# dalab/matrix-manifolds

Hardware: AMD Instinct MI355X
Metric: pairwise manifold-dist/sec (fwd+bwd), SPD(3) 5k-node (higher is better)
Workload: dtype f32; 1 GPU; grqc-class graph, n=5000 nodes -> SPD(3) affine-invariant, all 12497500 pairs, squared distance + backward, reference init (||log X||=0.1); parallelism=pair-rows sharded x1, 1 all-reduce, launch=hipGraph replay (kernels)

## Files before the change

matrix-manifolds_amd/csrc/smallmat.hpp:

```cpp
#pragma once
#include <hip/hip_runtime.h>

#include <cstdint>
#include <type_traits>
#include <utility>

namespace mm {

template <int D> struct Packed { static constexpr int NP = D * (D + 1) / 2; };

__host__ __device__ constexpr int pidx(int r, int c) {
  return r >= c ? r * (r + 1) / 2 + c : c * (c + 1) / 2 + r;
}

template <typename T> struct Num;
template <> struct Num<float> {
  static __device__ __forceinline__ float eps() { return 5.9604645e-8f; }
  static __device__ __forceinline__ float tiny() { return 1e-37f; }
  static __device__ __forceinline__ float sqrt(float x) { return __builtin_amdgcn_sqrtf(x); }
  static __device__ __forceinline__ float rsqrt(float x) { return __builtin_amdgcn_rsqf(x); }
  static __device__ __forceinline__ float rcp(float x) { return __builtin_amdgcn_rcpf(x); }
  static __device__ __forceinline__ float rcp_fast(float x) { return __builtin_amdgcn_rcpf(x); }
  static __device__ __forceinline__ float log(float x) { return __builtin_amdgcn_logf(x) * 0.6931471805599453f; }
  static __device__ __forceinline__ float exp(float x) { return ::expf(x); }
// ... 318 lines not shown
        const T apq = a[pidx(q, p)];
        const T h = a[pidx(q, q)] - a[pidx(p, p)];
        const T ah = N::abs(h) + T(1e-15);
        const T sa_ = (h < T(0)) ? -apq : apq;
        const T sa2 = sa_ + sa_;
        const T r = N::rsqrt(N::fma(ah, ah, sa2 * sa2));
        const T x = N::fma(ah * r, T(0.5), T(0.5));
        const T ci = N::rsqrt(x);
        const T c = x * ci;
        const T s = (sa_ * r) * ci;
        const T t = s * ci;
        a[pidx(p, p)] = N::fma(-t, apq, a[pidx(p, p)]);
        a[pidx(q, q)] = N::fma(t, apq, a[pidx(q, q)]);
        a[pidx(q, p)] = T(0);
#pragma unroll
        for (int r2 = 0; r2 < D; ++r2) {
          if (r2 == p || r2 == q) continue;
          const T arp = a[pidx(r2, p)], arq = a[pidx(r2, q)];
          a[pidx(r2, p)] = N::fma(c, arp, -s * arq);
          a[pidx(r2, q)] = N::fma(s, arp, c * arq);
        }
        if (WITH_V) {
#pragma unroll
          for (int r2 = 0; r2 < D; ++r2) {
            const T vrp = v[r2][p], vrq = v[r2][q];
            v[r2][p] = N::fma(c, vrp, -s * vrq);
            v[r2][q] = N::fma(s, vrp, c * vrq);
          }
        }
      }
    }
  }
}
template <typename T, int D, bool WITH_V>
__device__ __forceinline__ void jacobi_eig(T (&a)[Packed<D>::NP], T (&v)[D][D]) {
  jacobi_eig<T, D, WITH_V>(a, v, Num<T>::eps() * Num<T>::eps());
}

template <typename T, int D, bool WITH_V>
__device__ __forceinline__ void svd_onesided(const T (&g)[D][D], T (&b)[D][D], T (&v)[D][D], T tol2) {
  using N = Num<T>;
#pragma unroll
  for (int r = 0; r < D; ++r)
#pragma unroll
    for (int c = 0; c < D; ++c) {
      b[r][c] = g[r][c];
      if (WITH_V) v[r][c] = (r == c) ? T(1) : T(0);
    }
  if constexpr (D == 1) return;
  for (int sweep = 0; sweep < N::kMaxSweeps + 4; ++sweep) {
    bool active = false;
#pragma unroll
    for (int p = 0; p < D - 1; ++p) {
#pragma unroll
      for (int q = p + 1; q < D; ++q) {
        T app = T(0), aqq = T(0), apq = T(0);
#pragma unroll
        for (int r = 0; r < D; ++r) {
          app = N::fma(b[r][p], b[r][p], app);
          aqq = N::fma(b[r][q], b[r][q], aqq);
          apq = N::fma(b[r][p], b[r][q], apq);
        }
        active = active || (apq * apq > tol2 * (app * aqq));
        const T h = aqq - app;
        const T ah = N::abs(h) + T(1e-15);
        const T sa_ = (h < T(0)) ? -apq : apq;
        const T sa2 = sa_ + sa_;
        const T rr = N::rsqrt(N::fma(ah, ah, sa2 * sa2));
        const T x = N::fma(ah * rr, T(0.5), T(0.5));
        const T ci = N::rsqrt(x);
        const T c = x * ci;
        const T sn = (sa_ * rr) * ci;
#pragma unroll
        for (int r = 0; r < D; ++r) {
          const T bp = b[r][p], bq = b[r][q];
          b[r][p] = N::fma(c, bp, -sn * bq);
          b[r][q] = N::fma(sn, bp, c * bq);
          if (WITH_V) {
            const T vp = v[r][p], vq = v[r][q];
            v[r][p] = N::fma(c, vp, -sn * vq);
            v[r][q] = N::fma(sn, vp, c * vq);
          }
        }
      }
    }
    if (!__any(active)) break;
  }
}

__device__ __forceinline__ void eig3_trig(const float (&a)[6], float (&w)[3]) {
  const float q = (a[pidx(0, 0)] + a[pidx(1, 1)] + a[pidx(2, 2)]) * (1.f / 3.f);
  const float b00 = a[pidx(0, 0)] - q, b11 = a[pidx(1, 1)] - q, b22 = a[pidx(2, 2)] - q;
  const float o10 = a[pidx(1, 0)], o20 = a[pidx(2, 0)], o21 = a[pidx(2, 1)];
  float p2 = fmaf(b00, b00, fmaf(b11, b11, b22 * b22));
  p2 = fmaf(2.f, fmaf(o10, o10, fmaf(o20, o20, o21 * o21)), p2) * (1.f / 6.f);
  const float ip = __builtin_amdgcn_rsqf(fmaxf(p2, 1e-30f));
  const float p = p2 * ip;
  const float c00 = b00 * ip, c11 = b11 * ip, c22 = b22 * ip, c10 = o10 * ip, c20 = o20 * ip, c21 = o21 * ip;
  float hd = c00 * fmaf(c11, c22, -c21 * c21) - c10 * fmaf(c10, c22, -c21 * c20) + c20 * fmaf(c10, c21, -c11 * c20);
  hd = fminf(fmaxf(0.5f * hd, -1.f), 1.f);
  const float ax = fabsf(hd);
  float pa = fmaf(-0.0012624911f, ax, 0.0066700901f);
  pa = fmaf(pa, ax, -0.0170881256f);
  pa = fmaf(pa, ax, 0.0308918810f);
  pa = fmaf(pa, ax, -0.0501743046f);
  pa = fmaf(pa, ax, 0.0889789874f);
  pa = fmaf(pa, ax, -0.2145988016f);
  pa = fmaf(pa, ax, 1.5707963050f);
  const float ac = __builtin_amdgcn_sqrtf(1.f - ax) * pa;
  const float phi = ((hd < 0.f) ? 3.14159265358979f - ac : ac) * (1.f / 3.f);
  const float z = phi * phi;
  float cs = fmaf(z, -2.7557319e-7f, 2.4801587e-5f);
  cs = fmaf(cs, z, -1.3888889e-3f);
  cs = fmaf(cs, z, 4.1666667e-2f);
  cs = fmaf(cs, z, -0.5f);
  cs = fmaf(cs, z, 1.f);
  float sn = fmaf(z, -2.5052108e-8f, 2.7557319e-6f);
  sn = fmaf(sn, z, -1.9841270e-4f);
  sn = fmaf(sn, z, 8.3333333e-3f);
  sn = fmaf(sn, z, -1.6666667e-1f);
  sn = fmaf(sn * z, phi, phi);
  const float r3s = 1.7320508f * sn;
  w[2] = fmaf(p, cs + cs, q);
  w[1] = fmaf(p, r3s - cs, q);
  w[0] = fmaf(p, -r3s - cs, q);
}

template <typename T> struct LogSeries;
template <> struct LogSeries<float> {
  static constexpr int kTerms = 8;
  static constexpr float kA[kTerms] = {9.999999337e-01f, -4.999999402e-01f, 3.333568549e-01f, -2.500212282e-01f,
                                       1.987095623e-01f, -1.655023071e-01f, 1.650813480e-01f, -1.450413880e-01f};
  static constexpr float at(int i) { return kA[i]; }
};
template <> struct LogSeries<double> {
  static constexpr int kTerms = 20;
  static constexpr double kA[kTerms] = {
    1.00000000000000000e+00, -4.99999999999999944e-01, 3.33333333333343085e-01, -2.50000000000014155e-01,
    1.99999999996232608e-01, -1.66666666663750795e-01, 1.42857143404437337e-01, -1.25000000386766896e-01,
    1.11111071374215928e-01, -9.99999703591583217e-02, 9.09107326619259803e-02, -8.33346464041358065e-02,
    7.68821017515587124e-02, -7.13938378893102243e-02, 6.72936081364212679e-02, -6.30553787420979894e-02,
    5.31216751520414421e-02, -5.03380364382464973e-02, 8.02156472153527783e-02, -7.58480457039158590e-02};
  static constexpr double at(int i) { return kA[i]; }
};

template <typename T> __device__ __forceinline__ T log_series3(const T (&a)[6], T (&m0)[6], T pre = T(1)) {
  using N = Num<T>;
  using S = LogSeries<T>;
  const T e00 = a[pidx(0, 0)] - T(1), e11 = a[pidx(1, 1)] - T(1), e22 = a[pidx(2, 2)] - T(1);
  const T e10 = a[pidx(1, 0)], e20 = a[pidx(2, 0)], e21 = a[pidx(2, 1)];
  const T f00 = N::fma(e00, e00, N::fma(e10, e10, e20 * e20));
  const T f11 = N::fma(e10, e10, N::fma(e11, e11, e21 * e21));
  const T f22 = N::fma(e20, e20, N::fma(e21, e21, e22 * e22));
  const T f10 = N::fma(e10, e00, N::fma(e11, e10, e21 * e20));
  const T f20 = N::fma(e20, e00, N::fma(e21, e10, e22 * e20));
  const T f21 = N::fma(e20, e10, N::fma(e21, e11, e22 * e21));
  const T tr2 = f00 + f11 + f22;
  const T s1 = e00 + e11 + e22;
  const T s2 = T(0.5) * N::fma(s1, s1, -tr2);
  const T s3 = e00 * N::fma(e11, e22, -e21 * e21) - e10 * N::fma(e10, e22, -e21 * e20) +
               e20 * N::fma(e10, e21, -e11 * e20);
  T a0, a1, a2;
  ring_horner3<T, S>(s1, s2, s3, a0, a1, a2);
  const T b0 = (a2 * s3) * pre, b1 = N::fma(-a2, s2, a0) * pre, b2 = N::fma(a2, s1, a1) * pre;
  m0[pidx(0, 0)] = N::fma(b2, f00, N::fma(b1, e00, b0));
  m0[pidx(1, 1)] = N::fma(b2, f11, N::fma(b1, e11, b0));
  m0[pidx(2, 2)] = N::fma(b2, f22, N::fma(b1, e22, b0));
  m0[pidx(1, 0)] = N::fma(b2, f10, b1 * e10);
  m0[pidx(2, 0)] = N::fma(b2, f20, b1 * e20);
  m0[pidx(2, 1)] = N::fma(b2, f21, b1 * e21);
  return tr2;
}

constexpr double kCentredGate3 = 0.6534;
template <typename T> struct LogSeriesWide;
template <> struct LogSeriesWide<float> {
  static constexpr int kTerms = 16;
  static constexpr float kA[kTerms] = {9.999999847e-01f, -4.999999854e-01f, 3.333378158e-01f, -2.500042795e-01f,
                                       1.997873233e-01f, -1.664636323e-01f, 1.466440033e-01f, -1.286147090e-01f,
                                       7.866430935e-02f, -6.903477397e-02f, 2.371349367e-01f, -2.228347962e-01f,
                                       -2.667691364e-01f, 2.562672116e-01f, 4.274908187e-01f, -4.061057313e-01f};
  static constexpr float at(int i) { return kA[i]; }
};
template <> struct LogSeriesWide<double> {
  static constexpr int kTerms = 36;
  static constexpr double kA[kTerms] = {
    0.999999999999999977, -0.499999999999999978, 0.333333333333367457, -0.250000000000033421,
    0.199999999991592943, -0.166666666658432825, 0.142857143675747047, -0.125000000801733994,
    0.111111069196670012, -0.0999999589496586145, 0.0909103925504135392, -0.0833346081274524372,
    0.0768964148318060428, -0.071402459598029521, 0.0670466571631664423, -0.0628721421125401977,
    0.054920735255657598, -0.0517334464941176604, 0.0821825618685663011, -0.0789393499687729317,
    -0.119544506131984601, 0.11824425305853179, 0.753586818196905653, -0.737031529750978713,
    -2.21838624927452971, 2.17293423563498954, 5.34587266623974133, -5.23378983222008806,
    -8.94716963622682544, 8.7602754349000368, 10.4325804141314891, -10.2127945466777319,
    -7.42237802920880408, 7.26540890455107326, 2.58226980159039129, -2.52672226697783483};
  static constexpr double at(int i) { return kA[i]; }
};
template <typename T> __device__ __forceinline__ bool centred_far3(const T (&a)[6]) {
  using N = Num<T>;
  const T mu = (a[pidx(0, 0)] + a[pidx(1, 1)] + a[pidx(2, 2)]) * T(1.0 / 3.0);
  const T d0 = a[pidx(0, 0)] - mu, d1 = a[pidx(1, 1)] - mu, d2 = a[pidx(2, 2)] - mu;
  const T off = N::fma(a[pidx(1, 0)], a[pidx(1, 0)], N::fma(a[pidx(2, 0)], a[pidx(2, 0)], a[pidx(2, 1)] * a[pidx(2, 1)]));
  const T dev = N::fma(d0, d0, N::fma(d1, d1, N::fma(d2, d2, off + off)));
  return !(dev <= T(kCentredGate3) * (mu * mu)) || !(mu > T(0));
}
template <typename T> __device__ __forceinline__ void log_series3_centred(const T (&a)[6], T (&m0)[6], T pre = T(1)) {
  using N = Num<T>;
  using S = LogSeriesWide<T>;
  const T mu = (a[pidx(0, 0)] + a[pidx(1, 1)] + a[pidx(2, 2)]) * T(1.0 / 3.0);
  const T rmu = N::rcp(mu);
  const T e00 = N::fma(a[pidx(0, 0)], rmu, T(-1)), e11 = N::fma(a[pidx(1, 1)], rmu, T(-1)), e22 = N::fma(a[pidx(2, 2)], rmu, T(-1));
  const T e10 = a[pidx(1, 0)] * rmu, e20 = a[pidx(2, 0)] * rmu, e21 = a[pidx(2, 1)] * rmu;
  const T f00 = N::fma(e00, e00, N::fma(e10, e10, e20 * e20));
  const T f11 = N::fma(e10, e10, N::fma(e11, e11, e21 * e21));
  const T f22 = N::fma(e20, e20, N::fma(e21, e21, e22 * e22));
  const T f10 = N::fma(e10, e00, N::fma(e11, e10, e21 * e20));
  const T f20 = N::fma(e20, e00, N::fma(e21, e10, e22 * e20));
  const T f21 = N::fma(e20, e10, N::fma(e21, e11, e22 * e21));
  const T s2 = T(-0.5) * (f00 + f11 + f22);
  const T s3 = e00 * N::fma(e11, e22, -e21 * e21) - e10 * N::fma(e10, e22, -e21 * e20) +
               e20 * N::fma(e10, e21, -e11 * e20);
  T a0, a1, a2;
  ring_horner3<T, S, true>(T(0), s2, s3, a0, a1, a2);
  const T logmu = N::log(mu);
  const T b0 = N::fma(a2, s3, logmu) * pre, b1 = N::fma(-a2, s2, a0) * pre, b2 = a1 * pre;
  m0[pidx(0, 0)] = N::fma(b2, f00, N::fma(b1, e00, b0));
  m0[pidx(1, 1)] = N::fma(b2, f11, N::fma(b1, e11, b0));
  m0[pidx(2, 2)] = N::fma(b2, f22, N::fma(b1, e22, b0));
  m0[pidx(1, 0)] = N::fma(b2, f10, b1 * e10);
  m0[pidx(2, 0)] = N::fma(b2, f20, b1 * e20);
  m0[pidx(2, 1)] = N::fma(b2, f21, b1 * e21);
}

template <typename T> struct LogSqSeriesWide;
template <> struct LogSqSeriesWide<float> {
  static constexpr int kTerms = 16;
  static constexpr float kQ[kTerms] = {9.999998930e-01f, -9.999998963e-01f, 9.166980138e-01f, -8.333637039e-01f,
                                       7.596244972e-01f, -6.985597554e-01f, 6.746606801e-01f, -6.295878238e-01f,
                                       3.395295792e-01f, -3.133767555e-01f, 1.520582314e+00f, -1.462563750e+00f,
                                       -1.927056128e+00f, 1.871837175e+00f, 2.893810986e+00f, -2.795949233e+00f};
  static constexpr float at(int i) { return kQ[i]; }
};
template <typename T> __device__ __forceinline__ T logsq_series3_centred(const T (&a)[6]) {
  using N = Num<T>;
  using S = LogSqSeriesWide<T>;
  const T mu = (a[pidx(0, 0)] + a[pidx(1, 1)] + a[pidx(2, 2)]) * T(1.0 / 3.0);
  const T rmu = N::rcp(mu);
  const T e00 = N::fma(a[pidx(0, 0)], rmu, T(-1)), e11 = N::fma(a[pidx(1, 1)], rmu, T(-1)), e22 = N::fma(a[pidx(2, 2)], rmu, T(-1));
  const T e10 = a[pidx(1, 0)] * rmu, e20 = a[pidx(2, 0)] * rmu, e21 = a[pidx(2, 1)] * rmu;
  T t2 = N::fma(e00, e00, N::fma(e11, e11, e22 * e22));
  t2 = N::fma(T(2), N::fma(e10, e10, N::fma(e20, e20, e21 * e21)), t2);
  const T s1 = e00 + e11 + e22;
  const T s2 = T(-0.5) * t2;
  const T s3 = e00 * N::fma(e11, e22, -e21 * e21) - e10 * N::fma(e10, e22, -e21 * e20) +
               e20 * N::fma(e10, e21, -e11 * e20);
  T h0, h1, h2;
  ring_horner3<T, S, true>(T(0), s2, s3, h0, h1, h2);
  const T core = N::fma(h2, T(0.5) * t2 * t2, N::fma(h1, T(3) * s3, h0 * t2));
  const T lmu = N::log(mu), ldet = N::log((T(1) + s1) + (s2 + s3));
  return N::fma(lmu, N::fma(T(3), lmu, ldet + ldet), core);
}

constexpr double kCayleyGate = 0.36;
template <typename T> __device__ __forceinline__ T frexp_t(T x, int* k);
template <> __device__ __forceinline__ float frexp_t<float>(float x, int* k) { return ::frexpf(x, k); }
template <> __device__ __forceinline__ double frexp_t<double>(double x, int* k) { return ::frexp(x, k); }
template <typename T> __device__ __forceinline__ T ldexp_t(T x, int k);
template <> __device__ __forceinline__ float ldexp_t<float>(float x, int k) { return ::ldexpf(x, k); }
template <> __device__ __forceinline__ double ldexp_t<double>(double x, int k) { return ::ldexp(x, k); }

template <typename T> struct CayleyP;
template <> struct CayleyP<float> {
  static constexpr int K = 6;
  static constexpr float c[K + 1] = {1.00000002318570891e+00f, 3.33327042495924375e-01f, 2.00274867564608688e-01f,
                                     1.38428695737667723e-01f, 1.44240977093542333e-01f, -3.05379184438951401e-02f,
                                     2.73482843603638170e-01f};
  static constexpr int kTerms = K + 1;
  static constexpr float at(int i) { return c[i]; }
};
template <> struct CayleyP<double> {
  static constexpr int K = 13;
  static constexpr double c[K + 1] = {9.99999999999997002e-01, 3.33333333336093829e-01, 1.99999999512113669e-01,
                                      1.42857176992888746e-01, 1.11109865194520263e-01, 9.09362522505209464e-02,
                                      7.65413194323763535e-02, 7.02835946952955759e-02, 3.51739351378960174e-02,
                                      1.60038305495638411e-01, -2.87332526616183470e-01, 7.35063731671786291e-01,
                                      -8.29196169410508666e-01, 5.70221868872885063e-01};
  static constexpr int kTerms = K + 1;
  static constexpr double at(int i) { return c[i]; }
};
constexpr double kCayleyNarrow = 0.16;
struct CayleyPn64 {
  static constexpr double c[10] = {0.999999999999997828, 0.333333333336045998, 0.199999999442592788, 0.142857187137109386,
                                   0.111109332105236778, 0.0909499162581166662, 0.0763574513803657068, 0.0714494792571264998,
                                   0.0350458696353453726, 0.113663386241058913};
  static constexpr int kTerms = 10;
  static constexpr double at(int i) { return c[i]; }
};
struct CayleyQn64 {
  static constexpr double c[11] = {1.00000000000000037, 0.666666666666100058, 0.511111111252317187, 0.419047605361109196,
                                   0.357460995535957299, 0.313015598858362064, 0.279652848994267891, 0.248774877825649445,
                                   0.25954346018603201, 0.0906375847139156082, 0.475855998018695552};
  static constexpr int kTerms = 11;
  static constexpr double at(int i) { return c[i]; }
};
template <typename T> __device__ __forceinline__ T cayley_scale(T mean, T* logmu) {
  int k;
  const T mant = frexp_t<T>(mean, &k);
  if (mant < T(0.70710678118654752)) k -= 1;
  *logmu = T(k) * T(0.69314718055994531);
  return ldexp_t<T>(T(1), -k);
}
template <typename T>
__device__ __forceinline__ void cayley3_spectrum(T s1, T s2, T s3, T& rD, T& z1, T& z2, T& z3, T& t1, T& t2, T& t3) {
  using N = Num<T>;
  const T s33 = T(3) * s3;
  rD = N::rcp_fast(N::fma(T(4), s1, T(8)) + N::fma(T(2), s2, s3));
  z1 = N::fma(T(4), s1 + s2, s33) * rD;
  z2 = N::fma(T(2), s2, s33) * rD;
  z3 = s3 * rD;
  t1 = N::fma(z1, z1, T(-2) * z2);
  t2 = N::fma(z2, z2, T(-2) * (z1 * z3));
  t3 = z3 * z3;
}
template <typename T> __device__ __forceinline__ T log_cayley3(const T (&a)[6], T (&m0)[6], T pre = T(1)) {
  using N = Num<T>;
  using P = CayleyP<T>;
  T logmu;
  const T r = cayley_scale<T>((a[0] + a[2] + a[5]) * T(1.0 / 3.0), &logmu);
  const T e00 = N::fma(a[0], r, T(-1)), e11 = N::fma(a[2], r, T(-1)), e22 = N::fma(a[5], r, T(-1));
  const T e10 = a[1] * r, e20 = a[3] * r, e21 = a[4] * r;
  const T f00 = N::fma(e00, e00, N::fma(e10, e10, e20 * e20));
  const T f11 = N::fma(e10, e10, N::fma(e11, e11, e21 * e21));
  const T f22 = N::fma(e20, e20, N::fma(e21, e21, e22 * e22));
  const T f10 = N::fma(e10, e00, N::fma(e11, e10, e21 * e20));
  const T f20 = N::fma(e20, e00, N::fma(e21, e10, e22 * e20));
  const T f21 = N::fma(e20, e10, N::fma(e21, e11, e22 * e21));
  const T s1 = e00 + e11 + e22;
  const T s2 = T(0.5) * N::fma(s1, s1, -(f00 + f11 + f22));
  const T s3 = e00 * N::fma(e11, e22, -e21 * e21) - e10 * N::fma(e10, e22, -e21 * e20) +
               e20 * N::fma(e10, e21, -e11 * e20);
  T rD, z1, z2, z3, t1, t2, t3;
  cayley3_spectrum<T>(s1, s2, s3, rD, z1, z2, z3, t1, t2, t3);
  T c0, c1, c2;
  if constexpr (std::is_same<T, double>::value) {
    if (!__any(!(t1 <= T(kCayleyNarrow)))) ring_horner3<T, CayleyPn64>(t1, t2, t3, c0, c1, c2);
    else ring_horner3<T, P>(t1, t2, t3, c0, c1, c2);
  } else {
    ring_horner3<T, P>(t1, t2, t3, c0, c1, c2);
  }
  T b0 = c2 * z3, b1 = N::fma(-c2, z2, c1), b2 = c2 * z1;
  {
    const T n0 = N::fma(b2, z3, c0), n1 = N::fma(-b2, z2, b0), n2 = N::fma(b2, z1, b1);
    b0 = n0; b1 = n1; b2 = n2;
  }
  {
    const T n0 = b2 * z3, n1 = N::fma(-b2, z2, b0), n2 = N::fma(b2, z1, b1);
    b0 = n0; b1 = n1; b2 = n2;
  }
  const T y0 = z3, y2 = T(-2) * rD, y1 = -(s1 + T(2)) * y2;
  const T q0 = y0 * y0, q1 = T(2) * (y0 * y1), q2 = N::fma(T(2) * y0, y2, y1 * y1), q3 = T(2) * (y1 * y2), q4 = y2 * y2;
  const T h2 = N::fma(s1, s1, -s2), h1 = N::fma(-s1, s2, s3), h0 = s1 * s3;
  const T w0 = N::fma(q4, h0, N::fma(q3, s3, q0));
  const T w1 = N::fma(q4, h1, N::fma(-q3, s2, q1));
  const T w2 = N::fma(q4, h2, N::fma(q3, s1, q2));
  const T p2 = pre + pre;
  const T g0 = N::fma(N::fma(b2, w0, N::fma(b1, y0, b0)), p2, logmu * pre);
  const T g1 = N::fma(b2, w1, b1 * y1) * p2;
  const T g2 = N::fma(b2, w2, b1 * y2) * p2;
  m0[0] = N::fma(g2, f00, N::fma(g1, e00, g0));
  m0[2] = N::fma(g2, f11, N::fma(g1, e11, g0));
  m0[5] = N::fma(g2, f22, N::fma(g1, e22, g0));
  m0[1] = N::fma(g2, f10, g1 * e10);
  m0[3] = N::fma(g2, f20, g1 * e20);
  m0[4] = N::fma(g2, f21, g1 * e21);
  return t1;
}

template <typename T> struct CayleyQ;
template <> struct CayleyQ<float> {
  static constexpr int K = 7;
  static constexpr float c[K + 1] = {0.999999990659938783f, 0.666669978862739941f, 0.510920481665167664f, 0.423174655546735851f,
                                     0.314332175292986808f, 0.551201736862719326f, -0.412567514510121138f, 1.17039095371423926f};
  static constexpr int kTerms = K + 1;
  static constexpr float at(int i) { return c[i]; }
};
template <> struct CayleyQ<double> {
  static constexpr int K = 15;
  static constexpr double c[K + 1] = {0.99999999999999987, 0.666666666666851142, 0.511111111067702619, 0.419047623073864087,
                                      0.35746012197040091, 0.313040831979712641, 0.279195466546191997, 0.254162482860379539,
                                      0.217779908930427374, 0.303497422045376885, -0.242356046115491071, 1.74002823450430709,
                                      -3.70667784316895825, 6.72451540777742607, -6.69607770346690423, 3.64458881905822882};
  static constexpr int kTerms = K + 1;
  static constexpr double at(int i) { return c[i]; }
};
template <typename T> __device__ __forceinline__ T logsq_cayley3(const T (&a)[6], T logdet_a, T* gate) {
  using N = Num<T>;
  using Q = CayleyQ<T>;
  T logmu;
  const T r = cayley_scale<T>((a[0] + a[2] + a[5]) * T(1.0 / 3.0), &logmu);
  const T e00 = N::fma(a[0], r, T(-1)), e11 = N::fma(a[2], r, T(-1)), e22 = N::fma(a[5], r, T(-1));
  const T e10 = a[1] * r, e20 = a[3] * r, e21 = a[4] * r;
  const T s1 = e00 + e11 + e22;
  T tr2 = N::fma(e00, e00, N::fma(e11, e11, e22 * e22));
  tr2 = N::fma(T(2), N::fma(e10, e10, N::fma(e20, e20, e21 * e21)), tr2);
  const T s2 = T(0.5) * N::fma(s1, s1, -tr2);
  const T s3 = e00 * N::fma(e11, e22, -e21 * e21) - e10 * N::fma(e10, e22, -e21 * e20) +
               e20 * N::fma(e10, e21, -e11 * e20);
  T rD, z1, z2, z3, t1, t2, t3;
  cayley3_spectrum<T>(s1, s2, s3, rD, z1, z2, z3, t1, t2, t3);
  *gate = t1;
  const T p1 = t1, p2 = N::fma(t1, p1, T(-2) * t2), p3 = N::fma(t1, p2, N::fma(-t2, p1, T(3) * t3));
  T c0, c1, c2;
  if constexpr (std::is_same<T, double>::value) {
    if (!__any(!(t1 <= T(kCayleyNarrow)))) ring_horner3<T, CayleyQn64>(t1, t2, t3, c0, c1, c2);
    else ring_horner3<T, Q>(t1, t2, t3, c0, c1, c2);
  } else {
    ring_horner3<T, Q>(t1, t2, t3, c0, c1, c2);
  }
  const T s = N::fma(c2, p3, N::fma(c1, p2, c0 * p1));
  return N::fma(logmu, N::fma(T(-3), logmu, logdet_a + logdet_a), T(4) * s);
}

template <typename T, int D>
__device__ __forceinline__ void sym_mul(const T (&x)[Packed<D>::NP], const T (&y)[Packed<D>::NP], T (&o)[Packed<D>::NP]) {
#pragma unroll
  for (int r = 0; r < D; ++r)
#pragma unroll
    for (int c = 0; c <= r; ++c) {
      T acc = x[pidx(r, 0)] * y[pidx(0, c)];
#pragma unroll
      for (int k = 1; k < D; ++k) acc = Num<T>::fma(x[pidx(r, k)], y[pidx(k, c)], acc);
      o[pidx(r, c)] = acc;
    }
}

template <typename T, int D, typename S, int G>
__device__ __forceinline__ void log_series_mat(const T (&e)[Packed<D>::NP], T (&m0)[Packed<D>::NP]) {
  using N = Num<T>;
  constexpr int NP = Packed<D>::NP, K = S::kTerms, NG = K / G;
  static_assert((G == 2 || G == 4) && K % G == 0 && NG >= 2, "whole groups");
  T pw[NP], e2[G == 4 ? NP : 1], e3[G == 4 ? NP : 1];
  if constexpr (G == 4) {
    sym_mul<T, D>(e, e, e2);
    sym_mul<T, D>(e, e2, e3);
    sym_mul<T, D>(e2, e2, pw);
  } else {
    sym_mul<T, D>(e, e, pw);
  }
  auto add_group = [&](T (&dst)[NP], int j, bool first) __attribute__((always_inline)) {
    const T c0 = S::kA[G * j], c1 = S::kA[G * j + 1];
    T c2 = T(0), c3 = T(0);
    if constexpr (G == 4) { c2 = S::kA[G * j + 2]; c3 = S::kA[G * j + 3]; }
#pragma unroll
    for (int k = 0; k < NP; ++k) {
      T v = first ? c1 * e[k] : N::fma(c1, e[k], dst[k]);
      if constexpr (G == 4) v = N::fma(c3, e3[k], N::fma(c2, e2[k], v));
      dst[k] = v;
    }
#pragma unroll
    for (int r = 0; r < D; ++r) dst[pidx(r, r)] += c0;
  };
  T acc[NP], t[NP];
  add_group(acc, NG - 1, true);
  constexpr int kSteps = NG - 1;
#pragma unroll 1
  for (int j = NG - 2; j >= (kSteps & 1); j -= 2) {
    sym_mul<T, D>(acc, pw, t);
    add_group(t, j, false);
    sym_mul<T, D>(t, pw, acc);
    add_group(acc, j - 1, false);
  }
  if constexpr (kSteps & 1) {
    sym_mul<T, D>(acc, pw, t);
    add_group(t, 0, false);
    sym_mul<T, D>(e, t, m0);
  } else {
    sym_mul<T, D>(e, acc, m0);
  }
}
template <typename T, int D, typename S> constexpr int series_group() {
  if (S::kTerms <= 8) return 2;
  if (sizeof(T) == 4) return D <= 7 ? 4 : 2;
  return (D == 5 || (D == 6 && S::kTerms <= 20)) ? 4 : 2;
}
template <typename T, int D> __device__ __forceinline__ void log_close_mat(const T (&a)[Packed<D>::NP], T (&m0)[Packed<D>::NP]) {
  T e[Packed<D>::NP];
#pragma unroll
  for (int k = 0; k < Packed<D>::NP; ++k) e[k] = a[k];
#pragma unroll
  for (int r = 0; r < D; ++r) e[pidx(r, r)] -= T(1);
  log_series_mat<T, D, LogSeries<T>, series_group<T, D, LogSeries<T>>()>(e, m0);
}
template <typename T, int D> __device__ __forceinline__ bool centred_far_mat(const T (&a)[Packed<D>::NP]) {
  using N = Num<T>;
  T tr = a[pidx(0, 0)];
#pragma unroll
  for (int r = 1; r < D; ++r) tr += a[pidx(r, r)];
  const T mu = tr * T(1.0 / D);
  T dg = T(0), off = T(0);
#pragma unroll
  for (int r = 0; r < D; ++r) {
    const T d = a[pidx(r, r)] - mu;
    dg = N::fma(d, d, dg);
#pragma unroll
    for (int c = 0; c < r; ++c) off = N::fma(a[pidx(r, c)], a[pidx(r, c)], off);
  }
  const T dev = N::fma(T(2), off, dg);
  return !(dev <= T(0.66 * 0.66 * D / (D - 1.0)) * (mu * mu)) || !(mu > T(0));
}
template <typename T, int D> __device__ __forceinline__ void log_centred_mat(const T (&a)[Packed<D>::NP], T (&m0)[Packed<D>::NP]) {
  using N = Num<T>;
  T tr = a[pidx(0, 0)];
#pragma unroll
  for (int r = 1; r < D; ++r) tr += a[pidx(r, r)];
  const T mu = tr * T(1.0 / D), rmu = N::rcp(mu);
  T e[Packed<D>::NP];
#pragma unroll
  for (int k = 0; k < Packed<D>::NP; ++k) e[k] = a[k] * rmu;
#pragma unroll
  for (int r = 0; r < D; ++r) e[pidx(r, r)] -= T(1);
  log_series_mat<T, D, LogSeriesWide<T>, series_group<T, D, LogSeriesWide<T>>()>(e, m0);
  const T lm = N::log(mu);
#pragma unroll
  for (int r = 0; r < D; ++r) m0[pidx(r, r)] += lm;
}

template <typename T> __device__ __forceinline__ T log_cayley4(const T (&a)[10], T (&m0)[10]) {
// ... 399 lines not shown
```

matrix-manifolds_amd/csrc/spd_pair.hpp:

```cpp
#pragma once
#include <hip/hip_runtime.h>

#include "../../include/mm_manifolds.h"
#include "prof.hpp"
#include <algorithm>
#include <climits>
#include <cstdint>
#include <cstdlib>
#include <type_traits>

#include "smallmat.hpp"
#include "loss.hpp"
#include "adam.hpp"
#include "spd_rules.hpp"

#include "spd_ws.hpp"
#include "spd_step.hpp"
#include "stamp.hpp"

namespace mm {

template <typename T, int D>
__device__ __forceinline__ void node_tables(const T (&xs)[Packed<D>::NP], int i, T* __restrict__ nodeL, T* __restrict__ nodeX,
                                            T* __restrict__ nodeC, int* __restrict__ bad, T* __restrict__ nodeLd,
// ... 166 lines not shown
    return p2;
  }
}
constexpr double kCloseGate = 0.09;
template <typename T, int D> __device__ __forceinline__ void log_close(const T (&a)[Packed<D>::NP], T (&m0)[Packed<D>::NP],
                                                                     T pre = T(1)) {
  if constexpr (D == 3) log_series3<T>(a, m0, pre); else log_series4<T>(a, m0, pre);
}
template <typename T, int D> __device__ __forceinline__ T log_cayley(const T (&a)[Packed<D>::NP], T (&m0)[Packed<D>::NP], T pre = T(1)) {
  if constexpr (D == 3) {
    return log_cayley3<T>(a, m0, pre);
  } else {
    const T gate = log_cayley4<T>(a, m0);
#pragma unroll
    for (int k = 0; k < Packed<D>::NP; ++k) m0[k] *= pre;
    return gate;
  }
}
template <typename T, int D> constexpr bool fwd_uses_logdet() {
  return D == 3 && std::is_same<T, double>::value;
}

__host__ __device__ inline bool spd_clamps_wide(double wmin, double wmax) { return wmin <= 1e-6 && wmax >= 1e6; }
template <int D, int LOSS> inline bool spd_clamps_supported(double wmin, double wmax) {
  return (D <= 2 && LOSS == MM_LOSS_NONE) || spd_clamps_wide(wmin, wmax);
}
template <typename T, int D, bool CHOL = false, bool HAS_LD = false, typename TL>
__device__ __forceinline__ T pair_value(const TL (&li)[Packed<D>::NP], const T (&xj)[Packed<D>::NP], T wmin, T wmax,
                                        T logdet_a = T(0)) {
  if constexpr (D == 3 && std::is_same<T, float>::value) {
    float a[6], w[3], v[3][3];
    pair_a<float, 3, CHOL>(li, xj, a);
    if (__builtin_expect(!__any(!(close_dev3<float>(a) <= float(kCloseGate))), 1)) {
      float e2;
      return logsq_series3<float>(a, &e2);
    }
    if (!__any(centred_far3<float>(a))) return logsq_series3_centred<float>(a);
    eig3_trig(a, w);
    const bool wide = !(w[0] * 32.f > w[2]);
    if (__any(wide)) {
      if constexpr (CHOL) {
        float lw[3];
        return pair_core<float, 3, false, true>(li, xj, wmin, wmax, w, lw, v);
      } else {
        jacobi_eig<float, 3, false, true>(a, v, Num<float>::eps());
        w[0] = a[pidx(0, 0)]; w[1] = a[pidx(1, 1)]; w[2] = a[pidx(2, 2)];
      }
    }
    float s = 0.f;
#pragma unroll
    for (int k = 0; k < 3; ++k) {
      const float l = Num<float>::log(fminf(fmaxf(w[k], wmin), wmax));
      s = fmaf(l, l, s);
    }
    return s;
  } else if constexpr (D == 3 || D == 4) {
    constexpr int NP = Packed<D>::NP;
    T a[NP], m0[NP];
    pair_a<T, D, CHOL>(li, xj, a);
    if constexpr (D == 3) {
      if (__builtin_expect(!__any(!(close_dev3<T>(a) <= T(kCloseGate))), 1)) {
        T e2;
        return logsq_series3<T>(a, &e2);
      }
      if constexpr (HAS_LD && fwd_uses_logdet<T, D>()) {
        T gate;
        const T sc = logsq_cayley3<T>(a, logdet_a, &gate);
        if (__builtin_expect(!__any(!(gate <= T(kCayleyGate))), 1)) return sc;
        T w[D], lw[D], v[D][D];
        return pair_core<T, D, false, CHOL>(li, xj, wmin, wmax, w, lw, v);
      }
    } else {
      if (__builtin_expect(!__any(!(close_gate<T, D>(a) <= T(kCloseGate))), 1)) return logsq_series4<T>(a);
      if constexpr (std::is_same<T, float>::value) {
        if (!__any(centred_far4<T>(a))) return logsq_series4_centred<T>(a);
      }
    }
    const T gate = log_cayley<T, D>(a, m0);
    if (__builtin_expect(!__any(!(gate <= T(kCayleyGate))), 1)) return frob2<T, D>(m0);
    T w[D], lw[D], v[D][D];
    return pair_core<T, D, false, CHOL>(li, xj, wmin, wmax, w, lw, v);
  } else if constexpr (D == 2 && CHOL) {
    T mlog[3];
    return log_pair2_chol<T>(li, xj, wmin, wmax, mlog);
  } else if constexpr (D >= 5) {
    constexpr int NP = Packed<D>::NP;
    T a[NP], m0[NP];
    pair_a<T, D, CHOL>(li, xj, a);
    if (__builtin_expect(!__any(!(close_gate<T, D>(a) <= T(kCloseGate))), 1)) {
      log_close_mat<T, D>(a, m0);
      return frob2<T, D>(m0);
    }
    if (!__any(centred_far_mat<T, D>(a))) {
      log_centred_mat<T, D>(a, m0);
      return frob2<T, D>(m0);
    }
    T w[D], lw[D], v[D][D];
    return pair_core<T, D, false, CHOL>(li, xj, wmin, wmax, w, lw, v);
  } else {
    T w[D], lw[D], v[D][D];
    return pair_core<T, D, false, CHOL>(li, xj, wmin, wmax, w, lw, v);
  }
}

constexpr int kSpd2FwdNC = 2, kSpd2BwdNC = 2;
template <typename T, int D> constexpr int pair_cols() { return (sizeof(T) == 4 && D == 2) ? kSpd2FwdNC : (sizeof(T) == 4 && D <= 3) ? 2 : ((sizeof(T) == 4 && D == 4) ? MM_SPD4_FWD_NC : 1); }
template <typename T, int D> constexpr int pair_cols_bwd() { return (sizeof(T) == 4 && D == 3) ? MM_SPD3_BWD_NC : (sizeof(T) == 4 && D == 2) ? kSpd2BwdNC : ((sizeof(T) == 4 && D == 4) ? MM_SPD4_BWD_NC : 1); }

template <typename T, int D, int TI, bool SQ>
__global__ __launch_bounds__(kBlock) void spd_pdist_fwd_kernel(const T* __restrict__ nodeL,
                                                               const T* __restrict__ nodeY ,
                                                               const T* __restrict__ nodeLd , int n, int row_begin,
                                                               int row_end, T wmin, T wmax, T* __restrict__ out) {
  constexpr int NP = Packed<D>::NP;
  constexpr int NC = pair_cols<T, D>();
  constexpr bool kLd = fwd_uses_logdet<T, D>();
  static_assert(TI % 2 == 0, "the row loop is unrolled twice");
  const TileId tile = fold_tile<TI, kBlock * NC>(n, row_begin, row_end);
  if (!tile.ok) return;
  const int i0 = tile.i0, i1 = min(i0 + TI, row_end);
  const int lane = threadIdx.x & 63;
  const int wave = __builtin_amdgcn_readfirstlane(threadIdx.x >> 6);
  const int wave_j0 = tile.jbase + wave * (64 * NC);
  if (wave_j0 + 64 * NC - 1 <= i0) return;
  int jv[NC];
  unsigned joff[NC];
  T xj[NC][NP], ldj[NC];
  static_for<NC>([&](auto qc) {
    constexpr int q = decltype(qc)::value;
    const int j = wave_j0 + 64 * q + lane;
    const bool jin = j < n;
    jv[q] = jin ? j : INT32_MIN;
    asm volatile("" : "+v"(jv[q]));
    joff[q] = unsigned(j) * unsigned(sizeof(T));
#pragma unroll
    for (int k = 0; k < NP; ++k) xj[q][k] = T(0);
#pragma unroll
    for (int k = 0; k < D; ++k) xj[q][pidx(k, k)] = T(1);
    ldj[q] = T(0);
    if (jin) {
#pragma unroll
      for (int k = 0; k < NP; ++k) xj[q][k] = nodeY[size_t(j) * NP + k];
      if constexpr (kLd) ldj[q] = nodeLd[j];
    }
  });
  const int64_t base = pair_off(n, row_begin);
  char* op = reinterpret_cast<char*>(out + (pair_off(n, i0) - base - i0 - 1));
  unsigned ostep = unsigned(n - i0 - 2) * unsigned(sizeof(T));
  unsigned roff = unsigned(i0) * unsigned(NP * sizeof(T));
  T lrow[2][NP], ldrow[2] = {T(0), T(0)};
#pragma unroll
  for (int k = 0; k < NP; ++k) lrow[0][k] = nodeL[size_t(i0) * NP + k];
  if constexpr (kLd) ldrow[0] = nodeLd[i0];
  for (int ib = i0; ib < i1; ib += 2) {
#pragma unroll
    for (int u = 0; u < 2; ++u) {
      const int irow = ib + u;
      const int ieff = (u == 0 || irow < i1) ? irow : INT32_MAX;
      roff += unsigned(NP * sizeof(T));
      asm volatile("" : "+s"(roff));
      const T* rowp = reinterpret_cast<const T*>(reinterpret_cast<const char*>(nodeL) + roff);
#pragma unroll
      for (int k = 0; k < NP; ++k) lrow[u ^ 1][k] = rowp[k];
      if constexpr (kLd) ldrow[u ^ 1] = nodeLd[irow + 1];
      const T (&li)[NP] = lrow[u];
      static_for<NC>([&](auto qc) {
        constexpr int q = decltype(qc)::value;
        T s = Num<T>::max_raw_s(pair_value<T, D, true, kLd>(li, xj[q], wmin, wmax, ldj[q] - ldrow[u]), wmin);
        if constexpr (!SQ) s = Num<T>::sqrt(s);
        asm volatile("" : "+v"(joff[q]));
        if (jv[q] > ieff) *reinterpret_cast<T*>(op + joff[q]) = s;
      });
      op += ostep;
      ostep -= unsigned(sizeof(T));
    }
  }
}

template <typename T, int LOSS>
__device__ __forceinline__ T upstream_of(T loaded, T dsq, bool valid, int squared, T wmin, T sp, const LossArgs<T>& la,
                                         T& loss_acc, T& ds_acc) {
  if constexpr (LOSS == MM_LOSS_NONE) {
    if (__builtin_expect(!squared, 0)) loaded *= T(0.5) * Num<T>::rsqrt(Num<T>::max(dsq, wmin));
    return loaded;
  } else {
    T dldm;
    const T l = loss_term<T, LOSS>(sp * dsq, loaded, la, dldm);
    loss_acc += valid ? l : T(0);
    ds_acc += valid ? dldm * dsq : T(0);
    return valid ? dldm * sp : T(0);
  }
}

__device__ __forceinline__ int batch_node(const int* __restrict__ idx32, size_t k, int n_total) {
  return int(min(unsigned(idx32[2 * k]), unsigned(n_total - 1)));
}

template <typename T>
__device__ __forceinline__ T pair_row_load(const T* __restrict__ g, int n, int64_t base, int row, int j) {
  const char* grow = reinterpret_cast<const char*>(g + (pair_off(n, row) - base - row - 1));
  const unsigned off = unsigned(min(max(j, row + 1), n - 1)) * unsigned(sizeof(T));
  return *reinterpret_cast<const T*>(grow + off);
}

template <typename T, int D, int TI, int LOSS, bool SQ, int NCX = 0, bool SUB = false>
__global__ __launch_bounds__((64 * bwd_waves<T, D>()), (bwd_min_waves_nc<T, D, NCX>())) void spd_pdist_bwd_kernel(const T* __restrict__ nodeLC ,
                                                               const T* __restrict__ nodeY ,
                                                               const T* __restrict__ g, int n, int row_begin,
                                                               int row_end, T wmin, T wmax,
                                                               T* __restrict__ accM, T* __restrict__ accS,
                                                               LossArgs<T> la,
                                                               const int64_t* __restrict__ idx, int n_total,
                                                               WalkShares shares, int* __restrict__ share_tab) {
  static_assert(!SUB || LOSS != MM_LOSS_NONE, "node minibatches exist for the fused objective only");
  const int ns = SUB ? n_total : n;
  const int* idx32 = reinterpret_cast<const int*>(idx);
  constexpr int NP = Packed<D>::NP;
  constexpr int NW = bwd_waves<T, D>();
  constexpr int NC = NCX ? NCX : pair_cols_bwd<T, D>();
  constexpr int squared = SQ ? 1 : 0;
  T sp = T(1), loss_acc = T(0), ds_acc = T(0);
  loss_resolve<T, LOSS>(la);
  if constexpr (LOSS != MM_LOSS_NONE) sp = softplus_of(la.scale_raw);
  static_assert(TI % 2 == 0, "the row loop is unrolled twice");
  __shared__ T redM[NW][TI][NP];
  __shared__ T colS[NW][NC][D * D][64];
  MM_SPD_STAMP_BEGIN();
  __builtin_amdgcn_s_setprio(3);
  const ColWalk walk(n, row_begin, row_end, 64 * NC);
  int cb, r, rem;
  shares.of_cached(walk, int(blockIdx.x), share_tab, cb, r, rem);
  const int lane = threadIdx.x & 63;
  const int wave = __builtin_amdgcn_readfirstlane(threadIdx.x >> 6);
  bool red_writer;
  const int red_slot = reduce_slot<NP>(lane, red_writer);
  const int64_t base = pair_off(n, row_begin);
  MM_SPD_STAMP_MARK(0);
  const int wave_rows = (rem + NW - 1) / NW;
  constexpr int kPrioLast = 4;
  const int prio_last = max(kPrioLast, wave_rows / 10);
  const int prio_stretch = max(wave_rows - prio_last, 3) / 3;
  int rows_left = prio_stretch;
  int phase = 0;
  __shared__ T redJunk[NW][64];
  T* red_ptr = red_writer ? &redM[wave][0][red_slot] : &redJunk[wave][lane];
  const int red_step = red_writer ? NP : 0;

  while (rem > 0) {
    const int jbase = cb * (64 * NC);
    int jv[NC];
    unsigned joff[NC];
    T xj[NC][NP], accJ[NC][D][D];
    static_for<NC>([&](auto qc) {
      constexpr int q = decltype(qc)::value;
      const int j = jbase + 64 * q + lane;
      const bool jin = j < n;
      jv[q] = jin ? j : INT32_MIN;
      asm volatile("" : "+v"(jv[q]));
      joff[q] = unsigned(min(j, n - 1)) * unsigned(sizeof(T));
      int jn = j;
      if constexpr (SUB) {
        jn = batch_node(idx32, size_t(min(j, n - 1)), n_total);
        joff[q] = unsigned(jn) * unsigned(sizeof(T));
      }
#pragma unroll
      for (int k = 0; k < NP; ++k) xj[q][k] = T(0);
#pragma unroll
      for (int k = 0; k < D; ++k) xj[q][pidx(k, k)] = T(1);
      if (jin) {
#pragma unroll
        for (int k = 0; k < NP; ++k) xj[q][k] = nodeY[size_t(jn) * NP + k];
      }
#pragma unroll
      for (int rr = 0; rr < D; ++rr)
#pragma unroll
        for (int c = 0; c < D; ++c) accJ[q][rr][c] = T(0);
    });
    const int hi = walk.hi(cb);
    const int slice_cap = max(TI, int(min(int64_t(1) << 20, (int64_t(1) << 31) / (int64_t(n) * int64_t(sizeof(T))))));
    while (rem > 0 && r < hi) {
      const int chunk = int(min(int64_t(min(hi - r, rem)), int64_t(NW) * slice_cap));
      const int tw = (chunk + NW - 1) / NW;
      const int i0 = min(r + wave * tw, r + chunk), i1 = min(i0 + tw, r + chunk);
      if (i0 < i1) {
        constexpr int kAhead = 2;
        static_assert(kAhead == 2, "the one padding row of the operand table covers one masked slot: further ahead, clamp roff");
        const int first_node = SUB ? __builtin_amdgcn_readfirstlane(batch_node(idx32, size_t(i0), n_total)) : i0;
        int next_node = SUB ? __builtin_amdgcn_readfirstlane(batch_node(idx32, size_t(min(i0 + 1, n - 1)), n_total)) : 0;
        unsigned roff = unsigned(first_node) * unsigned(2 * NP * sizeof(T));
        T lrow[kAhead][2 * NP];
#pragma unroll
        for (int k = 0; k < 2 * NP; ++k) lrow[0][k] = nodeLC[size_t(first_node) * (2 * NP) + k];
        const int glast = min(i1, walk.re) - 1;
        const int64_t gk = glast - i0;
        const unsigned gmax = unsigned((gk * (n - 2) - (int64_t(i0) * gk + gk * (gk - 1) / 2)) * int64_t(sizeof(T)));
        const char* gslice = reinterpret_cast<const char*>(g + (pair_off(n, i0) - base - i0 - 1));
        unsigned goff = 0, gstep = unsigned(n - i0 - 2) * unsigned(sizeof(T));
        unsigned jslice[NC];
        static_for<NC>([&](auto qc) {
          constexpr int q = decltype(qc)::value;
          jslice[q] = max(joff[q], unsigned(i0 + 1) * unsigned(sizeof(T)));
        });
        T gq[kAhead][NC];
        int req_row = i0, req_node = first_node;
        auto request = [&](T (&dst)[NC]) __attribute__((always_inline)) {
          if constexpr (SUB) {
            const char* grow = reinterpret_cast<const char*>(g) + size_t(req_node) * size_t(n_total) * sizeof(T);
            static_for<NC>([&](auto qc) {
              constexpr int q = decltype(qc)::value;
              dst[q] = *reinterpret_cast<const T*>(grow + joff[q]);
            });
            req_row = min(req_row + 1, glast);
            req_node = __builtin_amdgcn_readfirstlane(batch_node(idx32, size_t(req_row), n_total));
          } else {
            static_for<NC>([&](auto qc) {
              constexpr int q = decltype(qc)::value;
              asm volatile("" : "+v"(jslice[q]));
              dst[q] = *reinterpret_cast<const T*>(gslice + goff + jslice[q]);
            });
            goff = min(goff + gstep, gmax);
            gstep -= unsigned(sizeof(T));
          }
        };
#pragma unroll
        for (int u = 0; u < kAhead; ++u) request(gq[u]);
        MM_SPD_STAMP_MARK(1);
        for (int s0 = i0; s0 < i1; s0 += TI) {
        const int s1 = min(s0 + TI, i1);
        for (int ib = s0; ib < s1; ib += kAhead) {
// ... 794 lines not shown
```

Measured before the change: 168.3 billion pairs/s.

## Use cofactor identity for matrix log series and unmask interior pair tiles

Rewrites the 3x3 log-series evaluators so the matrix square E^2 is no longer formed. Cayley-Hamilton lets the off-diagonal terms be taken from the cofactor (adjugate) entries, which s3 and s2 already need, with the polynomial coefficients folded to match. This removes several FMAs per pair. Separately, the pair-distance row loop gets an unmasked variant for wave tiles that lie entirely above the diagonal and inside n, which avoids per-store comparisons at the cost of doubling that code path.

```diff
diff --git a/matrix-manifolds_amd/csrc/smallmat.hpp b/matrix-manifolds_amd/csrc/smallmat.hpp
--- a/matrix-manifolds_amd/csrc/smallmat.hpp
+++ b/matrix-manifolds_amd/csrc/smallmat.hpp
@@ -494,23 +494,24 @@
   const T f00 = N::fma(e00, e00, N::fma(e10, e10, e20 * e20));
   const T f11 = N::fma(e10, e10, N::fma(e11, e11, e21 * e21));
   const T f22 = N::fma(e20, e20, N::fma(e21, e21, e22 * e22));
-  const T f10 = N::fma(e10, e00, N::fma(e11, e10, e21 * e20));
-  const T f20 = N::fma(e20, e00, N::fma(e21, e10, e22 * e20));
-  const T f21 = N::fma(e20, e10, N::fma(e21, e11, e22 * e21));
   const T tr2 = f00 + f11 + f22;
+  const T c00 = N::fma(e11, e22, -e21 * e21);
+  const T c10 = N::fma(e21, e20, -e10 * e22);
+  const T c20 = N::fma(e10, e21, -e11 * e20);
+  const T c21 = N::fma(e10, e20, -e00 * e21);
   const T s1 = e00 + e11 + e22;
   const T s2 = T(0.5) * N::fma(s1, s1, -tr2);
-  const T s3 = e00 * N::fma(e11, e22, -e21 * e21) - e10 * N::fma(e10, e22, -e21 * e20) +
-               e20 * N::fma(e10, e21, -e11 * e20);
+  const T s3 = N::fma(e20, c20, N::fma(e10, c10, e00 * c00));
   T a0, a1, a2;
   ring_horner3<T, S>(s1, s2, s3, a0, a1, a2);
   const T b0 = (a2 * s3) * pre, b1 = N::fma(-a2, s2, a0) * pre, b2 = N::fma(a2, s1, a1) * pre;
+  const T k1 = N::fma(b2, s1, b1);
   m0[pidx(0, 0)] = N::fma(b2, f00, N::fma(b1, e00, b0));
   m0[pidx(1, 1)] = N::fma(b2, f11, N::fma(b1, e11, b0));
   m0[pidx(2, 2)] = N::fma(b2, f22, N::fma(b1, e22, b0));
-  m0[pidx(1, 0)] = N::fma(b2, f10, b1 * e10);
-  m0[pidx(2, 0)] = N::fma(b2, f20, b1 * e20);
-  m0[pidx(2, 1)] = N::fma(b2, f21, b1 * e21);
+  m0[pidx(1, 0)] = N::fma(b2, c10, k1 * e10);
+  m0[pidx(2, 0)] = N::fma(b2, c20, k1 * e20);
+  m0[pidx(2, 1)] = N::fma(b2, c21, k1 * e21);
   return tr2;
 }
 
@@ -553,25 +554,21 @@
   const T rmu = N::rcp(mu);
   const T e00 = N::fma(a[pidx(0, 0)], rmu, T(-1)), e11 = N::fma(a[pidx(1, 1)], rmu, T(-1)), e22 = N::fma(a[pidx(2, 2)], rmu, T(-1));
   const T e10 = a[pidx(1, 0)] * rmu, e20 = a[pidx(2, 0)] * rmu, e21 = a[pidx(2, 1)] * rmu;
-  const T f00 = N::fma(e00, e00, N::fma(e10, e10, e20 * e20));
-  const T f11 = N::fma(e10, e10, N::fma(e11, e11, e21 * e21));
-  const T f22 = N::fma(e20, e20, N::fma(e21, e21, e22 * e22));
-  const T f10 = N::fma(e10, e00, N::fma(e11, e10, e21 * e20));
-  const T f20 = N::fma(e20, e00, N::fma(e21, e10, e22 * e20));
-  const T f21 = N::fma(e20, e10, N::fma(e21, e11, e22 * e21));
-  const T s2 = T(-0.5) * (f00 + f11 + f22);
-  const T s3 = e00 * N::fma(e11, e22, -e21 * e21) - e10 * N::fma(e10, e22, -e21 * e20) +
-               e20 * N::fma(e10, e21, -e11 * e20);
+  const T c00 = N::fma(e11, e22, -e21 * e21), c11 = N::fma(e00, e22, -e20 * e20), c22 = N::fma(e00, e11, -e10 * e10);
+  const T c10 = N::fma(e21, e20, -e10 * e22), c20 = N::fma(e10, e21, -e11 * e20), c21 = N::fma(e10, e20, -e00 * e21);
+  const T s2 = c00 + c11 + c22;
+  const T s3 = N::fma(e20, c20, N::fma(e10, c10, e00 * c00));
   T a0, a1, a2;
   ring_horner3<T, S, true>(T(0), s2, s3, a0, a1, a2);
   const T logmu = N::log(mu);
-  const T b0 = N::fma(a2, s3, logmu) * pre, b1 = N::fma(-a2, s2, a0) * pre, b2 = a1 * pre;
-  m0[pidx(0, 0)] = N::fma(b2, f00, N::fma(b1, e00, b0));
-  m0[pidx(1, 1)] = N::fma(b2, f11, N::fma(b1, e11, b0));
-  m0[pidx(2, 2)] = N::fma(b2, f22, N::fma(b1, e22, b0));
-  m0[pidx(1, 0)] = N::fma(b2, f10, b1 * e10);
-  m0[pidx(2, 0)] = N::fma(b2, f20, b1 * e20);
-  m0[pidx(2, 1)] = N::fma(b2, f21, b1 * e21);
+  const T b1 = N::fma(-a2, s2, a0) * pre, b2 = a1 * pre;
+  const T b0 = N::fma(-b2, s2, N::fma(a2, s3, logmu) * pre);
+  m0[pidx(0, 0)] = N::fma(b2, c00, N::fma(b1, e00, b0));
+  m0[pidx(1, 1)] = N::fma(b2, c11, N::fma(b1, e11, b0));
+  m0[pidx(2, 2)] = N::fma(b2, c22, N::fma(b1, e22, b0));
+  m0[pidx(1, 0)] = N::fma(b2, c10, b1 * e10);
+  m0[pidx(2, 0)] = N::fma(b2, c20, b1 * e20);
+  m0[pidx(2, 1)] = N::fma(b2, c21, b1 * e21);
 }
 
 template <typename T> struct LogSqSeriesWide;
@@ -671,16 +668,11 @@
   const T r = cayley_scale<T>((a[0] + a[2] + a[5]) * T(1.0 / 3.0), &logmu);
   const T e00 = N::fma(a[0], r, T(-1)), e11 = N::fma(a[2], r, T(-1)), e22 = N::fma(a[5], r, T(-1));
   const T e10 = a[1] * r, e20 = a[3] * r, e21 = a[4] * r;
-  const T f00 = N::fma(e00, e00, N::fma(e10, e10, e20 * e20));
-  const T f11 = N::fma(e10, e10, N::fma(e11, e11, e21 * e21));
-  const T f22 = N::fma(e20, e20, N::fma(e21, e21, e22 * e22));
-  const T f10 = N::fma(e10, e00, N::fma(e11, e10, e21 * e20));
-  const T f20 = N::fma(e20, e00, N::fma(e21, e10, e22 * e20));
-  const T f21 = N::fma(e20, e10, N::fma(e21, e11, e22 * e21));
+  const T c00 = N::fma(e11, e22, -e21 * e21), c11 = N::fma(e00, e22, -e20 * e20), c22 = N::fma(e00, e11, -e10 * e10);
+  const T c10 = N::fma(e21, e20, -e10 * e22), c20 = N::fma(e10, e21, -e11 * e20), c21 = N::fma(e10, e20, -e00 * e21);
   const T s1 = e00 + e11 + e22;
-  const T s2 = T(0.5) * N::fma(s1, s1, -(f00 + f11 + f22));
-  const T s3 = e00 * N::fma(e11, e22, -e21 * e21) - e10 * N::fma(e10, e22, -e21 * e20) +
-               e20 * N::fma(e10, e21, -e11 * e20);
+  const T s2 = c00 + c11 + c22;
+  const T s3 = N::fma(e20, c20, N::fma(e10, c10, e00 * c00));
   T rD, z1, z2, z3, t1, t2, t3;
   cayley3_spectrum<T>(s1, s2, s3, rD, z1, z2, z3, t1, t2, t3);
   T c0, c1, c2;
@@ -709,12 +701,13 @@
   const T g0 = N::fma(N::fma(b2, w0, N::fma(b1, y0, b0)), p2, logmu * pre);
   const T g1 = N::fma(b2, w1, b1 * y1) * p2;
   const T g2 = N::fma(b2, w2, b1 * y2) * p2;
-  m0[0] = N::fma(g2, f00, N::fma(g1, e00, g0));
-  m0[2] = N::fma(g2, f11, N::fma(g1, e11, g0));
-  m0[5] = N::fma(g2, f22, N::fma(g1, e22, g0));
-  m0[1] = N::fma(g2, f10, g1 * e10);
-  m0[3] = N::fma(g2, f20, g1 * e20);
-  m0[4] = N::fma(g2, f21, g1 * e21);
+  const T k0 = N::fma(-g2, s2, g0), k1 = N::fma(g2, s1, g1);
+  m0[0] = N::fma(g2, c00, N::fma(k1, e00, k0));
+  m0[2] = N::fma(g2, c11, N::fma(k1, e11, k0));
+  m0[5] = N::fma(g2, c22, N::fma(k1, e22, k0));
+  m0[1] = N::fma(g2, c10, k1 * e10);
+  m0[3] = N::fma(g2, c20, k1 * e20);
+  m0[4] = N::fma(g2, c21, k1 * e21);
   return t1;
 }
 
diff --git a/matrix-manifolds_amd/csrc/spd_pair.hpp b/matrix-manifolds_amd/csrc/spd_pair.hpp
--- a/matrix-manifolds_amd/csrc/spd_pair.hpp
+++ b/matrix-manifolds_amd/csrc/spd_pair.hpp
@@ -342,6 +342,9 @@
 #pragma unroll
   for (int k = 0; k < NP; ++k) lrow[0][k] = nodeL[size_t(i0) * NP + k];
   if constexpr (kLd) ldrow[0] = nodeLd[i0];
+  const bool interior = wave_j0 >= i1 && wave_j0 + 64 * NC <= n && ((i1 - i0) & 1) == 0;
+  auto row_loop = [&](auto masked_c) __attribute__((always_inline)) {
+  constexpr bool kMasked = decltype(masked_c)::value;
   for (int ib = i0; ib < i1; ib += 2) {
 #pragma unroll
     for (int u = 0; u < 2; ++u) {
@@ -359,12 +362,14 @@
         T s = Num<T>::max_raw_s(pair_value<T, D, true, kLd>(li, xj[q], wmin, wmax, ldj[q] - ldrow[u]), wmin);
         if constexpr (!SQ) s = Num<T>::sqrt(s);
         asm volatile("" : "+v"(joff[q]));
-        if (jv[q] > ieff) *reinterpret_cast<T*>(op + joff[q]) = s;
+        if (!kMasked || jv[q] > ieff) *reinterpret_cast<T*>(op + joff[q]) = s;
       });
       op += ostep;
       ostep -= unsigned(sizeof(T));
     }
   }
+  };
+  if (interior) row_loop(std::false_type{}); else row_loop(std::true_type{});
 }
 
 template <typename T, int LOSS>
```

Measured after the change: 171.8 billion pairs/s, median of 6. 2.1% higher.
